# tzt101/MichiGAN

Hardware: AMD Instinct MI355X
Metric: training images/sec at 512x512 (G+D step) (higher is better)
Workload: dtype bf16; 1 GPU; SPADEB G + multiscale PatchGAN D + VGG19 + Gabor orientation losses, full G step + D step (Adam), bs=8/GPU, 512x512, BASELINE.json configs[2]; global_batch=8, batch_per_gpu=8, resolution=512, parallelism=dp1, init=reference default (xavier, 0.02), random VGG weights

## Files before the change

### michigan_amd/csrc/mg_wgrad3x3.hip

```cpp
#include "mg_conv_common.h"
#include "mg_wgrad_common.h"


namespace {

typedef __attribute__((ext_vector_type(4))) short s16x4_t;
typedef __attribute__((ext_vector_type(8))) short s16x8_t;
typedef __attribute__((address_space(3))) s16x4_t* lds_s16x4_p;

__device__ unsigned long long* g_mg_wg3_probe_out = nullptr;
__device__ __forceinline__ unsigned long long wg3_stamp()
{
    unsigned long long v;
    asm volatile("s_memrealtime %0\n\ts_waitcnt lgkmcnt(0)" : "=s"(v) :: "memory");
    return v;
}

template <int MT, int NT, bool W16, bool PROBE = false>
__global__ __launch_bounds__(256, 2) void wgrad3x3_kernel(const Wg3K d)
{
    constexpr int TM = 64 * MT, TN = 64 * NT;
    constexpr int RBA = TM * 2, RBB = TN * 2;
    constexpr int PPA = RBA / 16, PPB = RBB / 16;
    constexpr int A_ROWS = 32, B_ROWS = (NT == 2) ? 36 : 40;
    constexpr int A_BYTES = A_ROWS * RBA, B_BYTES = B_ROWS * RBB;
    constexpr int A_IPS = A_BYTES / 4096;
    constexpr int B_IPS = (B_BYTES + 4095) / 4096;
    constexpr int IPS = A_IPS + B_IPS;
    constexpr int STAGE = A_BYTES + B_BYTES;
    constexpr int NS = 4;
    static_assert(A_BYTES % 4096 == 0 && B_BYTES % 1024 == 0, "stage must be whole wave blocks");

    extern __shared__ __attribute__((aligned(16))) unsigned char smem[];

    const int tid = threadIdx.x, lane = tid & 63;
    const int wave = __builtin_amdgcn_readfirstlane(tid >> 6);
    const int wm = wave >> 1, wn = wave & 1;
    const int l31 = lane & 31, hi = lane >> 5;

    int tile;
    {
        const int nblk = gridDim.x, b = blockIdx.x;
        const int q8 = nblk >> 3, r8 = nblk & 7, xcd = b & 7, idx = b >> 3;
        tile = (xcd < r8 ? xcd * (q8 + 1) : r8 * (q8 + 1) + (xcd - r8) * q8) + idx;
    }
    const int tm = tile % d.tiles_m;  tile /= d.tiles_m;
    const int tn = tile % d.tiles_n;  tile /= d.tiles_n;
    const int ky = tile % 3;
    const int split = tile / 3;
    const int m0 = tm * TM, n0 = tn * TN;
    const int sbeg = split * d.sps;
    const int send = min(d.nstg, sbeg + d.sps);
    const int nk = send - sbeg;
    if (nk <= 0) return;

    const int H = d.H, W = d.W;
    constexpr int SEG = W16 ? 16 : 32, SEGP = SEG + 2;
    constexpr int PR = (32 / SEG) * SEGP;
    const unsigned lds0 = (unsigned)(size_t)(__attribute__((address_space(3))) unsigned char*)smem;
    const unsigned dump = lds0 + NS * STAGE + wave * 1024;
    const unsigned char* zsrc = g_mg_zeros + (lane & 3) * 16;

    auto swz_a = [](int row) { return RBA == 256 ? (row & 3) : ((row >> 1) & 1); };
    auto swz_b = [](int row) { return RBB == 256 ? (row & 3) : ((row >> 1) & 1); };

    int aoff[A_IPS];
#pragma unroll
    for (int j = 0; j < A_IPS; ++j) {
        const int g = j * 256 + tid, row = g / PPA, slot = g % PPA;
        int ch = m0 + ((slot ^ (swz_a(row) << 2)) << 3);
        if (ch >= d.Cg) ch = m0;
        aoff[j] = (row * d.Cg + ch) * 2;
    }
    int boff[B_IPS], brc[B_IPS];
#pragma unroll
    for (int j = 0; j < B_IPS; ++j) {
        const int g = j * 256 + tid, row = g / PPB, slot = g % PPB;
        int ch = n0 + ((slot ^ (swz_b(row) << 2)) << 3);
        if (ch >= d.Cin) ch = n0;
        const int r = (W16 && row >= SEGP) ? 1 : 0, c = row - r * SEGP - 1;
        boff[j] = (((r + ky - 1) * W + c) * d.Cin + ch) * 2;
        brc[j] = row < PR ? (r | (c + 1) << 4) : -1;
    }
    const unsigned char* const dy0 = reinterpret_cast<const unsigned char*>(d.dy);
    const unsigned char* const x0p = reinterpret_cast<const unsigned char*>(d.x);
    const unsigned char* abase; const unsigned char* xbase;
    int sy, sx, sg_next = sbeg;
    int simg = 0, sstripe = 0;
    const int SWp = W16 ? W : d.stripe_w, nsegs = SWp / 32, nstripes = W / SWp;
    if (W16) {
        abase = dy0 + (size_t)sbeg * 32 * d.Cg * 2;
        xbase = x0p + (size_t)sbeg * 32 * d.Cin * 2;
        const int rem = (sbeg * 32) % (H * W); sy = rem / W; sx = rem - sy * W;
    } else {
        const int spi = H * (W / 32);
        simg = sbeg / spi;
        int r = sbeg - simg * spi;
        sstripe = r / (H * nsegs);  r -= sstripe * (H * nsegs);
        sy = r / nsegs;
        sx = sstripe * SWp + (r - sy * nsegs) * 32;
        const size_t p = ((size_t)simg * H + sy) * W + sx;
        abase = dy0 + p * d.Cg * 2;
        xbase = x0p + p * d.Cin * 2;
    }
    sy = __builtin_amdgcn_readfirstlane(sy); sx = __builtin_amdgcn_readfirstlane(sx);
    simg = __builtin_amdgcn_readfirstlane(simg); sstripe = __builtin_amdgcn_readfirstlane(sstripe);
    const int a_step = 32 * d.Cg * 2, x_step = 32 * d.Cin * 2;

    unsigned long long m_live[B_IPS], m_left[B_IPS], m_right[B_IPS], m_r1[B_IPS];
#pragma unroll
    for (int j = 0; j < B_IPS; ++j) {
        const bool lv = brc[j] >= 0;
        const int c = (brc[j] >> 4) - 1, r = brc[j] & 15;
        m_live[j]  = __builtin_amdgcn_ballot_w64(lv);
        m_left[j]  = __builtin_amdgcn_ballot_w64(lv && c == -1);
        m_right[j] = __builtin_amdgcn_ballot_w64(lv && c == SEG);
        m_r1[j]    = __builtin_amdgcn_ballot_w64(lv && r == 1);
    }
    const unsigned long long zaddr = (unsigned long long)(size_t)zsrc;
    const unsigned zlo = (unsigned)zaddr, zhi = (unsigned)(zaddr >> 32);

    auto issue = [&](int stage) {
        const bool real = sg_next < send;
        const unsigned sbase = lds0 + stage * STAGE;
        if (real) {
#pragma unroll
            for (int j = 0; j < A_IPS; ++j)
                glds16_s(abase, (unsigned)aoff[j], __builtin_amdgcn_readfirstlane(sbase + j * 4096 + wave * 1024));
        } else {
#pragma unroll
            for (int j = 0; j < A_IPS; ++j)
                glds16(zsrc, __builtin_amdgcn_readfirstlane(sbase + j * 4096 + wave * 1024));
        }
        const int sxs = __builtin_amdgcn_readfirstlane(sx), sys = __builtin_amdgcn_readfirstlane(sy), kys = __builtin_amdgcn_readfirstlane(ky);
        const bool lok = sxs > 0, rok = sxs + SEG < W;
        const bool y0 = (unsigned)(sys + kys - 1) < (unsigned)H, y1 = (unsigned)(sys + kys) < (unsigned)H;
#pragma unroll
        for (int j = 0; j < B_IPS; ++j) {
            unsigned long long v = real ? m_live[j] : 0ull;
            if (!lok) v &= ~m_left[j];
            if (!rok) v &= ~m_right[j];
            if (W16) { if (!y0) v &= m_r1[j]; if (!y1) v &= ~m_r1[j]; }
            else if (!y0) v = 0ull;
            v = ((unsigned long long)(unsigned)__builtin_amdgcn_readfirstlane((int)(v >> 32)) << 32) | (unsigned)__builtin_amdgcn_readfirstlane((int)v);
            asm("" : "+s"(v));
            const unsigned long long pa = (unsigned long long)(size_t)(xbase + boff[j]);
            unsigned plo, phi;
            asm("v_cndmask_b32_e64 %0, %1, %2, %3" : "=v"(plo) : "v"(zlo), "v"((unsigned)pa), "s"(v));
            asm("v_cndmask_b32_e64 %0, %1, %2, %3" : "=v"(phi) : "v"(zhi), "v"((unsigned)(pa >> 32)), "s"(v));
            const bool live = (j * 4096 + wave * 1024) < B_BYTES;
            glds16(reinterpret_cast<const void*>((size_t)(((unsigned long long)phi << 32) | plo)),
                   __builtin_amdgcn_readfirstlane(live ? sbase + A_BYTES + j * 4096 + wave * 1024 : dump));
        }
        ++sg_next;
        if (W16) {
            abase += a_step; xbase += x_step;
            sy += 2; if (sy >= H) sy = 0;
        } else {
            sx += 32;
            if (sx < (sstripe + 1) * SWp) { abase += a_step; xbase += x_step; }
            else {
                sx = sstripe * SWp; ++sy;
                if (sy >= H) { sy = 0; ++sstripe; if (sstripe >= nstripes) { sstripe = 0; ++simg; } sx = sstripe * SWp; }
                const size_t p = ((size_t)simg * H + sy) * W + sx;
                abase = dy0 + p * d.Cg * 2;
                xbase = x0p + p * d.Cin * 2;
            }
        }
    };

    f32x16_t acc[3][MT][NT];
#pragma unroll
    for (int kx = 0; kx < 3; ++kx)
#pragma unroll
        for (int mt = 0; mt < MT; ++mt)
#pragma unroll
            for (int nt = 0; nt < NT; ++nt)
#pragma unroll
                for (int r = 0; r < 16; ++r) acc[kx][mt][nt][r] = 0.f;

    const bool do_bias = d.dbias != nullptr && ky == 1 && tn == 0 && wn == 0;
    float bsum[MT];
#pragma unroll
    for (int mt = 0; mt < MT; ++mt) bsum[mt] = 0.f;

    const int i16 = lane & 15, g2 = lane >> 4;
    const int rsub = (g2 >> 1) * 8 + (i16 >> 2);
    const int csub = ((g2 & 1) * 16 + (i16 & 3) * 4) * 2;
    constexpr int ksb = W16 ? SEGP : 16;

    auto compute = [&](int slot) {
        const unsigned char* As = smem + slot * STAGE;
        const unsigned char* Bs = As + A_BYTES;
#pragma unroll
        for (int ks = 0; ks < 2; ++ks) {
            bf16x8_t a[MT];
            const int ra = ks * 16 + rsub;
#pragma unroll
            for (int mt = 0; mt < MT; ++mt) {
                const int col = ((wm * MT + mt) * 64 + csub) ^ (swz_a(ra) << 6);
                const unsigned char* p = As + ra * RBA + col;
                s16x4_t v0 = __builtin_amdgcn_ds_read_tr16_b64_v4i16((lds_s16x4_p)(p));
                s16x4_t v1 = __builtin_amdgcn_ds_read_tr16_b64_v4i16((lds_s16x4_p)(p + 4 * RBA));
                a[mt] = __builtin_bit_cast(bf16x8_t, __builtin_shufflevector(v0, v1, 0, 1, 2, 3, 4, 5, 6, 7));
                if (do_bias) {
                    typedef __attribute__((ext_vector_type(4))) unsigned u32x4_t;
                    const u32x4_t w = __builtin_bit_cast(u32x4_t, a[mt]);
#pragma unroll
                    for (int j = 0; j < 4; ++j) bsum[mt] += __uint_as_float(w[j] << 16) + __uint_as_float(w[j] & 0xffff0000u);
                }
            }
            static_for<0, 3>([&](auto kx_) {
                constexpr int kx = decltype(kx_)::value;
                bf16x8_t b[NT];
                const int rb = ks * ksb + kx + rsub;
#pragma unroll
                for (int nt = 0; nt < NT; ++nt) {
                    const int col = ((wn * NT + nt) * 64 + csub) ^ (swz_b(rb) << 6);
                    const unsigned char* p = Bs + rb * RBB + col;
                    s16x4_t v0 = __builtin_amdgcn_ds_read_tr16_b64_v4i16((lds_s16x4_p)(p));
                    s16x4_t v1 = __builtin_amdgcn_ds_read_tr16_b64_v4i16((lds_s16x4_p)(p + 4 * RBB));
                    b[nt] = __builtin_bit_cast(bf16x8_t, __builtin_shufflevector(v0, v1, 0, 1, 2, 3, 4, 5, 6, 7));
                }
#pragma unroll
                for (int mt = 0; mt < MT; ++mt)
#pragma unroll
                    for (int nt = 0; nt < NT; ++nt)
                        acc[kx][mt][nt] = __builtin_amdgcn_mfma_f32_32x32x16_bf16(a[mt], b[nt], acc[kx][mt][nt], 0, 0, 0);
            });
        }
    };

#pragma unroll
    for (int s = 0; s < NS - 1; ++s) issue(s);
    int slot = 0, islot = NS - 1;
    unsigned long long t_wait = 0, t_bar = 0, t_issue = 0, t_mfma = 0, t_begin = 0;
    if constexpr (PROBE) t_begin = wg3_stamp();
    for (int it = 0; it < nk; ++it) {
        unsigned long long s0 = 0, s1 = 0, s2 = 0, s3 = 0;
        if constexpr (PROBE) s0 = wg3_stamp();
        wait_vmcnt<(NS - 2) * IPS>();
        if constexpr (PROBE) s1 = wg3_stamp();
        __builtin_amdgcn_s_barrier();
        if constexpr (PROBE) s2 = wg3_stamp();
        issue(islot);
        if constexpr (PROBE) s3 = wg3_stamp();
        compute(slot);
        if constexpr (PROBE) { const unsigned long long s4 = wg3_stamp(); t_wait += s1 - s0; t_bar += s2 - s1; t_issue += s3 - s2; t_mfma += s4 - s3; }
        slot = (slot == NS - 1) ? 0 : slot + 1;
        islot = (islot == NS - 1) ? 0 : islot + 1;
    }
    wait_vmcnt<0>();
    unsigned long long t_loop_end = 0;
    if constexpr (PROBE) t_loop_end = wg3_stamp();

    if (do_bias) {
#pragma unroll
        for (int mt = 0; mt < MT; ++mt) {
            const float t = bsum[mt] + __shfl_xor(bsum[mt], 32);
            const int co = m0 + (wm * MT + mt) * 32 + l31;
            if (hi == 0 && co < d.Cg) wg_accum(d.dbias, d.det_stride, split, (size_t)co, t);
        }
    }

    static_for<0, 3 * MT * NT>([&](auto i_) {
        constexpr int kx = decltype(i_)::value / (MT * NT), mt = (decltype(i_)::value / NT) % MT, nt = decltype(i_)::value % NT;
        const int ci = n0 + (wn * NT + nt) * 32 + l31;
        if (ci >= d.Cin) return;
        const int tap = ky * 3 + kx;
#pragma unroll
        for (int r = 0; r < 16; ++r) {
            const int co = m0 + (wm * MT + mt) * 32 + (r & 3) + 8 * (r >> 2) + 4 * hi;
            if (co < d.Cg)
                wg_accum(d.dw, d.det_stride, split, (size_t)(tap * d.Cg + co) * d.Cin + ci, acc[kx][mt][nt][r]);
        }
    });
    if constexpr (PROBE) {
        const unsigned long long t_end = wg3_stamp();
        if (lane == 0 && g_mg_wg3_probe_out) {
            unsigned long long* o = g_mg_wg3_probe_out + ((size_t)blockIdx.x * 4 + wave) * 8;
            o[0] = t_wait; o[1] = t_bar; o[2] = t_issue; o[3] = t_mfma; o[4] = t_loop_end - t_begin; o[5] = t_end - t_loop_end; o[6] = (unsigned long long)nk; o[7] = t_begin;
        }
    }
}


template <int MT, int NT, bool W16>
int launch3(Wg3K& k, hipStream_t st, int* nsplit, bool dry)
{
    constexpr int TM = 64 * MT, TN = 64 * NT;
    constexpr int STAGE = 32 * TM * 2 + ((NT == 2) ? 36 : 40) * TN * 2;
    constexpr size_t LDS = 4 * (size_t)STAGE + 4096;
    k.tiles_m = (k.Cg + TM - 1) / TM;
    k.tiles_n = (k.Cin + TN - 1) / TN;
    const int stripe = mg_opt(MG_OPT_WGRAD3X3_STRIPE);
    k.stripe_w = (!W16 && stripe >= 32 && (stripe % 32) == 0 && k.W > stripe && (k.W % stripe) == 0) ? stripe : k.W;
    const long base = 3L * k.tiles_m * k.tiles_n;
    int S = k.splitk;
    if (S <= 0) {
        const int lo = (int)((384 + base - 1) / base), hi = (int)((1536 + base - 1) / base);
        S = k.nstg / 192 < hi ? k.nstg / 192 : hi;
        if (S < lo) S = lo;
        if (S > k.nstg / 16) S = k.nstg / 16;
        if (S < 1) S = 1;
    }
    if (S > k.nstg) S = k.nstg;
    k.sps = (k.nstg + S - 1) / S;
    S = (k.nstg + k.sps - 1) / k.sps;
    const long nblk = base * S;
    if (nsplit) *nsplit = S;
    if (dry) return MG_OK;
    if (nblk <= 0 || nblk > 0x7fffffffL) return mg_fail(MG_ERR_ARG, "mg_conv_wgrad: bad grid %ld", nblk);
    auto kern = wgrad3x3_kernel<MT, NT, W16>;
    constexpr size_t LDS_HALF_CU = LDS > 84 * 1024 ? LDS : 84 * 1024;
    const size_t lds_req = k.half_cu ? LDS_HALF_CU : LDS;
    mg_raise_lds_cap(reinterpret_cast<const void*>(kern), (int)LDS_HALF_CU);
#if MG_PROBES
    if constexpr (MT == 2 && NT == 2 && !W16) {
        if (mg_opt(MG_OPT_PROBE_WGRAD3X3)) {
            auto pk = wgrad3x3_kernel<MT, NT, W16, true>;
            mg_raise_lds_cap(reinterpret_cast<const void*>(pk), (int)LDS);
            hipLaunchKernelGGL(pk, dim3((unsigned)nblk), dim3(256), LDS, st, k);
            MG_CHECK_LAUNCH("mg_conv_wgrad(3x3 probe)");
            return MG_OK;
        }
    }
#endif
    hipLaunchKernelGGL(kern, dim3((unsigned)nblk), dim3(256), lds_req, st, k);
    MG_CHECK_LAUNCH("mg_conv_wgrad(3x3)");
    return MG_OK;
}

}

int wgrad3x3_set_probe(unsigned long long addr)
{
    unsigned long long* p = reinterpret_cast<unsigned long long*>(addr);
    return hipMemcpyToSymbol(HIP_SYMBOL(g_mg_wg3_probe_out), &p, sizeof(p)) == hipSuccess ? MG_OK : MG_ERR_ARG;
}

int launch_wgrad3x3(Wg3K& k, hipStream_t st, int* nsplit, bool dry)
{
    const bool m2 = k.Cg > 64, n2 = k.Cin > 64;
    if (k.W == 16) {
        if (m2 && n2) return launch3<2, 2, true>(k, st, nsplit, dry);
        if (m2)       return launch3<2, 1, true>(k, st, nsplit, dry);
        if (n2)       return launch3<1, 2, true>(k, st, nsplit, dry);
        return launch3<1, 1, true>(k, st, nsplit, dry);
    }
    if (m2 && n2) return launch3<2, 2, false>(k, st, nsplit, dry);
    if (m2)       return launch3<2, 1, false>(k, st, nsplit, dry);
    if (n2)       return launch3<1, 2, false>(k, st, nsplit, dry);
    return launch3<1, 1, false>(k, st, nsplit, dry);
}
```

Before: 131.8 images/s.

## Add nine-tap 3x3 weight-gradient kernel reusing input rows across ky taps

For W != 16, 3x3 weight-gradient convolutions now go to a new kernel. Each block computes all nine taps for a 64x64 tile. Input rows stream through a ring of LDS stages, so the three ky taps reuse the previous, current and next rows already in LDS, and the kx shift is formed in registers with alignbit instead of separate loads. This removes the separate grid dimension over ky and the threefold reloading of x and dy. The cost is nine accumulator tiles per wave (high register pressure), a fixed 64x64 tile, and a different split-K heuristic.

```diff
diff --git a/michigan_amd/csrc/mg_wgrad3x3.hip b/michigan_amd/csrc/mg_wgrad3x3.hip
--- a/michigan_amd/csrc/mg_wgrad3x3.hip
+++ b/michigan_amd/csrc/mg_wgrad3x3.hip
@@ -7,6 +7,7 @@
 typedef __attribute__((ext_vector_type(4))) short s16x4_t;
 typedef __attribute__((ext_vector_type(8))) short s16x8_t;
 typedef __attribute__((address_space(3))) s16x4_t* lds_s16x4_p;
+typedef __attribute__((ext_vector_type(4))) unsigned u32x4_t;
 
 __device__ unsigned long long* g_mg_wg3_probe_out = nullptr;
 __device__ __forceinline__ unsigned long long wg3_stamp()
@@ -16,7 +17,258 @@
     return v;
 }
 
-template <int MT, int NT, bool W16, bool PROBE = false>
+template <int RB>
+__device__ __forceinline__ bf16x8_t wg3_frag(const unsigned char* p)
+{
+    s16x4_t v0 = __builtin_amdgcn_ds_read_tr16_b64_v4i16((lds_s16x4_p)(p));
+    s16x4_t v1 = __builtin_amdgcn_ds_read_tr16_b64_v4i16((lds_s16x4_p)(p + 4 * RB));
+    return __builtin_bit_cast(bf16x8_t, __builtin_shufflevector(v0, v1, 0, 1, 2, 3, 4, 5, 6, 7));
+}
+
+__device__ __forceinline__ float wg3_sum8(bf16x8_t a)
+{
+    const u32x4_t w = __builtin_bit_cast(u32x4_t, a);
+    float s = 0.f;
+#pragma unroll
+    for (int j = 0; j < 4; ++j) s += __uint_as_float(w[j] << 16) + __uint_as_float(w[j] & 0xffff0000u);
+    return s;
+}
+
+__device__ __forceinline__ int wg3_tile()
+{
+    const int nblk = gridDim.x, b = blockIdx.x;
+    const int q8 = nblk >> 3, r8 = nblk & 7, xcd = b & 7, idx = b >> 3;
+    return (xcd < r8 ? xcd * (q8 + 1) : r8 * (q8 + 1) + (xcd - r8) * q8) + idx;
+}
+
+struct Wg9 {
+    static constexpr int RB = 128;
+    static constexpr int A_BYTES = 32 * RB;
+    static constexpr int B_BYTES = 40 * RB;
+    static constexpr int STAGE = A_BYTES + B_BYTES;
+    static constexpr int IPS = 3;
+    static constexpr int PF = 3;
+    static constexpr int NS = PF + 3;
+    static constexpr int DUMP = NS * STAGE, ZERO = DUMP + 4096;
+    static constexpr int LDS = ZERO + B_BYTES;
+};
+
+template <bool PROBE>
+__global__ __launch_bounds__(256, 2) void wgrad3x3_ninetap_kernel(const Wg3K d)
+{
+    constexpr int RB = Wg9::RB, A_BYTES = Wg9::A_BYTES, B_BYTES = Wg9::B_BYTES, STAGE = Wg9::STAGE, NS = Wg9::NS, PF = Wg9::PF;
+    constexpr int LIVE = 34;
+
+    extern __shared__ __attribute__((aligned(16))) unsigned char smem[];
+
+    const int tid = threadIdx.x, lane = tid & 63;
+    const int wave = __builtin_amdgcn_readfirstlane(tid >> 6);
+    const int wm = wave >> 1, wn = wave & 1;
+    const int l31 = lane & 31, hi = lane >> 5;
+
+    int tile = wg3_tile();
+    const int tm = tile % d.tiles_m;  tile /= d.tiles_m;
+    const int tn = tile % d.tiles_n;
+    const int split = tile / d.tiles_n;
+    const int m0 = tm * 64, n0 = tn * 64;
+    const int sbeg = split * d.sps;
+    const int send = min(d.nstg, sbeg + d.sps);
+    const int nk = send - sbeg;
+    if (nk <= 0) return;
+
+    const int H = d.H, W = d.W, nstripes = W / 32;
+    const unsigned lds0 = (unsigned)(size_t)(__attribute__((address_space(3))) unsigned char*)smem;
+    const unsigned dump = lds0 + Wg9::DUMP + wave * 1024;
+    const unsigned char* zsrc = g_mg_zeros + (lane & 3) * 16;
+
+    auto swz = [](int row) { return (row >> 1) & 1; };
+
+    int aoff, boff[2];
+    bool blive[2];
+    {
+        const int row = tid >> 3, slot = tid & 7;
+        int ch = m0 + ((slot ^ (swz(row) << 2)) << 3);
+        if (ch >= d.Cg) ch = m0;
+        aoff = (row * d.Cg + ch) * 2;
+    }
+#pragma unroll
+    for (int j = 0; j < 2; ++j) {
+        const int g = j * 256 + tid, row = g >> 3, slot = g & 7;
+        int ch = n0 + ((slot ^ (swz(row) << 2)) << 3);
+        if (ch >= d.Cin) ch = n0;
+        boff[j] = ((row - 1) * d.Cin + ch) * 2;
+        blive[j] = row < LIVE;
+    }
+    unsigned long long m_live[2], m_left[2], m_right[2];
+#pragma unroll
+    for (int j = 0; j < 2; ++j) {
+        const int row = (j * 256 + tid) >> 3;
+        m_live[j]  = __builtin_amdgcn_ballot_w64(blive[j]);
+        m_left[j]  = __builtin_amdgcn_ballot_w64(blive[j] && row == 0);
+        m_right[j] = __builtin_amdgcn_ballot_w64(blive[j] && row == LIVE - 1);
+    }
+    const unsigned long long zaddr = (unsigned long long)(size_t)zsrc;
+    const unsigned zlo = (unsigned)zaddr, zhi = (unsigned)(zaddr >> 32);
+
+    const unsigned char* const dy0 = reinterpret_cast<const unsigned char*>(d.dy);
+    const unsigned char* const x0p = reinterpret_cast<const unsigned char*>(d.x);
+    const int a_row = W * d.Cg * 2, x_row = W * d.Cin * 2;
+    int an = sbeg, ay, astripe, aimg;
+    int xs = sbeg - 1, xy, xstripe, ximg;
+    const int xlast = min(send, d.nstg - 1);
+    {
+        int is = sbeg / H;
+        ay = sbeg - is * H; aimg = is / nstripes; astripe = is - aimg * nstripes;
+        const int x1 = max(xs, 0);
+        is = x1 / H;
+        xy = x1 - is * H; ximg = is / nstripes; xstripe = is - ximg * nstripes;
+    }
+    ay = __builtin_amdgcn_readfirstlane(ay); astripe = __builtin_amdgcn_readfirstlane(astripe); aimg = __builtin_amdgcn_readfirstlane(aimg);
+    xy = __builtin_amdgcn_readfirstlane(xy); xstripe = __builtin_amdgcn_readfirstlane(xstripe); ximg = __builtin_amdgcn_readfirstlane(ximg);
+    const unsigned char* abase = dy0 + (((size_t)aimg * H + ay) * W + astripe * 32) * d.Cg * 2;
+    const unsigned char* xbase = x0p + (((size_t)ximg * H + xy) * W + xstripe * 32) * d.Cin * 2;
+
+    auto issue_a = [&](unsigned sbase) {
+        const unsigned dst = __builtin_amdgcn_readfirstlane(sbase + wave * 1024);
+        if (an < send) glds16_s(abase, (unsigned)aoff, dst);
+        else glds16(zsrc, dst);
+        ++an; ++ay;
+        if (ay < H) abase += a_row;
+        else {
+            ay = 0; ++astripe;
+            if (astripe >= nstripes) { astripe = 0; ++aimg; }
+            abase = dy0 + ((size_t)aimg * H * W + astripe * 32) * d.Cg * 2;
+        }
+    };
+    auto issue_b = [&](unsigned bbase) {
+        const bool real = xs >= 0 && xs <= xlast;
+        const int sxs = __builtin_amdgcn_readfirstlane(xstripe) * 32;
+        const bool lok = sxs > 0, rok = sxs + 32 < W;
+#pragma unroll
+        for (int j = 0; j < 2; ++j) {
+            unsigned long long v = real ? m_live[j] : 0ull;
+            if (!lok) v &= ~m_left[j];
+            if (!rok) v &= ~m_right[j];
+            v = ((unsigned long long)(unsigned)__builtin_amdgcn_readfirstlane((int)(v >> 32)) << 32) | (unsigned)__builtin_amdgcn_readfirstlane((int)v);
+            asm("" : "+s"(v));
+            const unsigned long long pa = (unsigned long long)(size_t)(xbase + boff[j]);
+            unsigned plo, phi;
+            asm("v_cndmask_b32_e64 %0, %1, %2, %3" : "=v"(plo) : "v"(zlo), "v"((unsigned)pa), "s"(v));
+            asm("v_cndmask_b32_e64 %0, %1, %2, %3" : "=v"(phi) : "v"(zhi), "v"((unsigned)(pa >> 32)), "s"(v));
+            const bool inside = (j * 4096 + wave * 1024) < B_BYTES;
+            glds16(reinterpret_cast<const void*>((size_t)(((unsigned long long)phi << 32) | plo)),
+                   __builtin_amdgcn_readfirstlane(inside ? bbase + j * 4096 + wave * 1024 : dump));
+        }
+        if (real) {
+            ++xy;
+            if (xy < H) xbase += x_row;
+            else {
+                xy = 0; ++xstripe;
+                if (xstripe >= nstripes) { xstripe = 0; ++ximg; }
+                xbase = x0p + ((size_t)ximg * H * W + xstripe * 32) * d.Cin * 2;
+            }
+        }
+        ++xs;
+    };
+
+    f32x16_t acc[9];
+#pragma unroll
+    for (int t = 0; t < 9; ++t)
+#pragma unroll
+        for (int r = 0; r < 16; ++r) acc[t][r] = 0.f;
+
+    const bool do_bias = d.dbias != nullptr && tn == 0 && wn == 0;
+    float bsum = 0.f;
+
+    const int i16 = lane & 15, g2 = lane >> 4;
+    const int rsub = (g2 >> 1) * 8 + (i16 >> 2);
+    const int csub = ((g2 & 1) * 16 + (i16 & 3) * 4) * 2;
+
+    auto compute = [&](const unsigned char* As, const unsigned char* B0, const unsigned char* B1, const unsigned char* B2) {
+#pragma unroll
+        for (int ks = 0; ks < 2; ++ks) {
+            const int ra = ks * 16 + rsub;
+            const bf16x8_t a = wg3_frag<RB>(As + ra * RB + ((wm * 64 + csub) ^ (swz(ra) << 6)));
+            if (do_bias) bsum += wg3_sum8(a);
+            static_for<0, 3>([&](auto ky_) {
+                constexpr int ky = decltype(ky_)::value;
+                const unsigned char* Bs = ky == 0 ? B0 : ky == 1 ? B1 : B2;
+                const int r0 = ks * 16 + rsub, r2 = r0 + 2;
+                const bf16x8_t b0 = wg3_frag<RB>(Bs + r0 * RB + ((wn * 64 + csub) ^ (swz(r0) << 6)));
+                const bf16x8_t b2 = wg3_frag<RB>(Bs + r2 * RB + ((wn * 64 + csub) ^ (swz(r2) << 6)));
+                const u32x4_t u0 = __builtin_bit_cast(u32x4_t, b0), u2 = __builtin_bit_cast(u32x4_t, b2);
+                u32x4_t u1;
+#pragma unroll
+                for (int i = 0; i < 4; ++i) u1[i] = __builtin_amdgcn_alignbit(i < 3 ? u0[(i + 1) & 3] : u2[3], u0[i], 16);
+                acc[ky * 3 + 0] = __builtin_amdgcn_mfma_f32_32x32x16_bf16(a, b0, acc[ky * 3 + 0], 0, 0, 0);
+                acc[ky * 3 + 1] = __builtin_amdgcn_mfma_f32_32x32x16_bf16(a, __builtin_bit_cast(bf16x8_t, u1), acc[ky * 3 + 1], 0, 0, 0);
+                acc[ky * 3 + 2] = __builtin_amdgcn_mfma_f32_32x32x16_bf16(a, b2, acc[ky * 3 + 2], 0, 0, 0);
+            });
+        }
+    };
+
+    glds16(zsrc, __builtin_amdgcn_readfirstlane(lds0 + Wg9::ZERO + wave * 1024));
+    glds16(zsrc, __builtin_amdgcn_readfirstlane(wave == 0 ? lds0 + Wg9::ZERO + 4096 : dump));
+    issue_b(lds0 + 0 * STAGE + A_BYTES);
+    issue_b(lds0 + 1 * STAGE + A_BYTES);
+#pragma unroll
+    for (int s = 2; s < PF + 2; ++s) { issue_a(lds0 + s * STAGE); issue_b(lds0 + s * STAGE + A_BYTES); }
+    int s0 = 0, s1 = 1, s2 = 2, islot = NS - 1;
+    int cy = __builtin_amdgcn_readfirstlane(sbeg % H);
+    unsigned long long t_wait = 0, t_bar = 0, t_issue = 0, t_mfma = 0, t_begin = 0;
+    if constexpr (PROBE) t_begin = wg3_stamp();
+    for (int it = 0; it < nk; ++it) {
+        unsigned long long p0 = 0, p1 = 0, p2 = 0, p3 = 0;
+        if constexpr (PROBE) p0 = wg3_stamp();
+        wait_vmcnt<(PF - 1) * Wg9::IPS>();
+        if constexpr (PROBE) p1 = wg3_stamp();
+        __builtin_amdgcn_s_barrier();
+        if constexpr (PROBE) p2 = wg3_stamp();
+        issue_a(lds0 + islot * STAGE); issue_b(lds0 + islot * STAGE + A_BYTES);
+        if constexpr (PROBE) p3 = wg3_stamp();
+        const unsigned char* const zs = smem + Wg9::ZERO;
+        compute(smem + s2 * STAGE,
+                cy == 0 ? zs : smem + s0 * STAGE + A_BYTES,
+                smem + s1 * STAGE + A_BYTES,
+                cy == H - 1 ? zs : smem + s2 * STAGE + A_BYTES);
+        if constexpr (PROBE) { const unsigned long long p4 = wg3_stamp(); t_wait += p1 - p0; t_bar += p2 - p1; t_issue += p3 - p2; t_mfma += p4 - p3; }
+        s0 = s1; s1 = s2;
+        s2 = (s2 == NS - 1) ? 0 : s2 + 1;
+        islot = (islot == NS - 1) ? 0 : islot + 1;
+        cy = (cy == H - 1) ? 0 : cy + 1;
+    }
+    wait_vmcnt<0>();
+    unsigned long long t_loop_end = 0;
+    if constexpr (PROBE) t_loop_end = wg3_stamp();
+
+    if (do_bias) {
+        const float t = bsum + __shfl_xor(bsum, 32);
+        const int co = m0 + wm * 32 + l31;
+        if (hi == 0 && co < d.Cg) wg_accum(d.dbias, d.det_stride, split, (size_t)co, t);
+    }
+
+    const int ci = n0 + wn * 32 + l31;
+    if (ci < d.Cin) {
+        static_for<0, 9>([&](auto t_) {
+            constexpr int tap = decltype(t_)::value;
+#pragma unroll
+            for (int r = 0; r < 16; ++r) {
+                const int co = m0 + wm * 32 + (r & 3) + 8 * (r >> 2) + 4 * hi;
+                if (co < d.Cg)
+                    wg_accum(d.dw, d.det_stride, split, (size_t)(tap * d.Cg + co) * d.Cin + ci, acc[tap][r]);
+            }
+        });
+    }
+    if constexpr (PROBE) {
+        const unsigned long long t_end = wg3_stamp();
+        if (lane == 0 && g_mg_wg3_probe_out) {
+            unsigned long long* o = g_mg_wg3_probe_out + ((size_t)blockIdx.x * 4 + wave) * 8;
+            o[0] = t_wait; o[1] = t_bar; o[2] = t_issue; o[3] = t_mfma; o[4] = t_loop_end - t_begin; o[5] = t_end - t_loop_end; o[6] = (unsigned long long)nk; o[7] = t_begin;
+        }
+    }
+}
+
+template <int MT, int NT>
 __global__ __launch_bounds__(256, 2) void wgrad3x3_kernel(const Wg3K d)
 {
     constexpr int TM = 64 * MT, TN = 64 * NT;
@@ -38,12 +290,7 @@
     const int wm = wave >> 1, wn = wave & 1;
     const int l31 = lane & 31, hi = lane >> 5;
 
-    int tile;
-    {
-        const int nblk = gridDim.x, b = blockIdx.x;
-        const int q8 = nblk >> 3, r8 = nblk & 7, xcd = b & 7, idx = b >> 3;
-        tile = (xcd < r8 ? xcd * (q8 + 1) : r8 * (q8 + 1) + (xcd - r8) * q8) + idx;
-    }
+    int tile = wg3_tile();
     const int tm = tile % d.tiles_m;  tile /= d.tiles_m;
     const int tn = tile % d.tiles_n;  tile /= d.tiles_n;
     const int ky = tile % 3;
@@ -55,8 +302,8 @@
     if (nk <= 0) return;
 
     const int H = d.H, W = d.W;
-    constexpr int SEG = W16 ? 16 : 32, SEGP = SEG + 2;
-    constexpr int PR = (32 / SEG) * SEGP;
+    constexpr int SEG = 16, SEGP = SEG + 2;
+    constexpr int PR = 2 * SEGP;
     const unsigned lds0 = (unsigned)(size_t)(__attribute__((address_space(3))) unsigned char*)smem;
     const unsigned dump = lds0 + NS * STAGE + wave * 1024;
     const unsigned char* zsrc = g_mg_zeros + (lane & 3) * 16;
@@ -78,44 +325,23 @@
         const int g = j * 256 + tid, row = g / PPB, slot = g % PPB;
         int ch = n0 + ((slot ^ (swz_b(row) << 2)) << 3);
         if (ch >= d.Cin) ch = n0;
-        const int r = (W16 && row >= SEGP) ? 1 : 0, c = row - r * SEGP - 1;
+        const int r = row >= SEGP ? 1 : 0, c = row - r * SEGP - 1;
         boff[j] = (((r + ky - 1) * W + c) * d.Cin + ch) * 2;
         brc[j] = row < PR ? (r | (c + 1) << 4) : -1;
     }
-    const unsigned char* const dy0 = reinterpret_cast<const unsigned char*>(d.dy);
-    const unsigned char* const x0p = reinterpret_cast<const unsigned char*>(d.x);
-    const unsigned char* abase; const unsigned char* xbase;
-    int sy, sx, sg_next = sbeg;
-    int simg = 0, sstripe = 0;
-    const int SWp = W16 ? W : d.stripe_w, nsegs = SWp / 32, nstripes = W / SWp;
-    if (W16) {
-        abase = dy0 + (size_t)sbeg * 32 * d.Cg * 2;
-        xbase = x0p + (size_t)sbeg * 32 * d.Cin * 2;
-        const int rem = (sbeg * 32) % (H * W); sy = rem / W; sx = rem - sy * W;
-    } else {
-        const int spi = H * (W / 32);
-        simg = sbeg / spi;
-        int r = sbeg - simg * spi;
-        sstripe = r / (H * nsegs);  r -= sstripe * (H * nsegs);
-        sy = r / nsegs;
-        sx = sstripe * SWp + (r - sy * nsegs) * 32;
-        const size_t p = ((size_t)simg * H + sy) * W + sx;
-        abase = dy0 + p * d.Cg * 2;
-        xbase = x0p + p * d.Cin * 2;
-    }
-    sy = __builtin_amdgcn_readfirstlane(sy); sx = __builtin_amdgcn_readfirstlane(sx);
-    simg = __builtin_amdgcn_readfirstlane(simg); sstripe = __builtin_amdgcn_readfirstlane(sstripe);
+    const unsigned char* abase = reinterpret_cast<const unsigned char*>(d.dy) + (size_t)sbeg * 32 * d.Cg * 2;
+    const unsigned char* xbase = reinterpret_cast<const unsigned char*>(d.x) + (size_t)sbeg * 32 * d.Cin * 2;
+    int sy = ((sbeg * 32) % (H * W)) / W, sg_next = sbeg;
+    sy = __builtin_amdgcn_readfirstlane(sy);
     const int a_step = 32 * d.Cg * 2, x_step = 32 * d.Cin * 2;
 
-    unsigned long long m_live[B_IPS], m_left[B_IPS], m_right[B_IPS], m_r1[B_IPS];
+    unsigned long long m_live[B_IPS], m_r1[B_IPS];
 #pragma unroll
     for (int j = 0; j < B_IPS; ++j) {
-        const bool lv = brc[j] >= 0;
         const int c = (brc[j] >> 4) - 1, r = brc[j] & 15;
-        m_live[j]  = __builtin_amdgcn_ballot_w64(lv);
-        m_left[j]  = __builtin_amdgcn_ballot_w64(lv && c == -1);
-        m_right[j] = __builtin_amdgcn_ballot_w64(lv && c == SEG);
-        m_r1[j]    = __builtin_amdgcn_ballot_w64(lv && r == 1);
+        const bool lv = brc[j] >= 0 && c != -1 && c != SEG;
+        m_live[j] = __builtin_amdgcn_ballot_w64(lv);
+        m_r1[j]   = __builtin_amdgcn_ballot_w64(lv && r == 1);
     }
     const unsigned long long zaddr = (unsigned long long)(size_t)zsrc;
     const unsigned zlo = (unsigned)zaddr, zhi = (unsigned)(zaddr >> 32);
@@ -132,16 +358,13 @@
             for (int j = 0; j < A_IPS; ++j)
                 glds16(zsrc, __builtin_amdgcn_readfirstlane(sbase + j * 4096 + wave * 1024));
         }
-        const int sxs = __builtin_amdgcn_readfirstlane(sx), sys = __builtin_amdgcn_readfirstlane(sy), kys = __builtin_amdgcn_readfirstlane(ky);
-        const bool lok = sxs > 0, rok = sxs + SEG < W;
+        const int sys = __builtin_amdgcn_readfirstlane(sy), kys = __builtin_amdgcn_readfirstlane(ky);
         const bool y0 = (unsigned)(sys + kys - 1) < (unsigned)H, y1 = (unsigned)(sys + kys) < (unsigned)H;
 #pragma unroll
         for (int j = 0; j < B_IPS; ++j) {
             unsigned long long v = real ? m_live[j] : 0ull;
-            if (!lok) v &= ~m_left[j];
-            if (!rok) v &= ~m_right[j];
-            if (W16) { if (!y0) v &= m_r1[j]; if (!y1) v &= ~m_r1[j]; }
-            else if (!y0) v = 0ull;
+            if (!y0) v &= m_r1[j];
+            if (!y1) v &= ~m_r1[j];
             v = ((unsigned long long)(unsigned)__builtin_amdgcn_readfirstlane((int)(v >> 32)) << 32) | (unsigned)__builtin_amdgcn_readfirstlane((int)v);
             asm("" : "+s"(v));
             const unsigned long long pa = (unsigned long long)(size_t)(xbase + boff[j]);
@@ -153,20 +376,8 @@
                    __builtin_amdgcn_readfirstlane(live ? sbase + A_BYTES + j * 4096 + wave * 1024 : dump));
         }
         ++sg_next;
-        if (W16) {
-            abase += a_step; xbase += x_step;
-            sy += 2; if (sy >= H) sy = 0;
-        } else {
-            sx += 32;
-            if (sx < (sstripe + 1) * SWp) { abase += a_step; xbase += x_step; }
-            else {
-                sx = sstripe * SWp; ++sy;
-                if (sy >= H) { sy = 0; ++sstripe; if (sstripe >= nstripes) { sstripe = 0; ++simg; } sx = sstripe * SWp; }
-                const size_t p = ((size_t)simg * H + sy) * W + sx;
-                abase = dy0 + p * d.Cg * 2;
-                xbase = x0p + p * d.Cin * 2;
-            }
-        }
+        abase += a_step; xbase += x_step;
+        sy += 2; if (sy >= H) sy = 0;
     };
 
     f32x16_t acc[3][MT][NT];
@@ -187,7 +398,7 @@
     const int i16 = lane & 15, g2 = lane >> 4;
     const int rsub = (g2 >> 1) * 8 + (i16 >> 2);
     const int csub = ((g2 & 1) * 16 + (i16 & 3) * 4) * 2;
-    constexpr int ksb = W16 ? SEGP : 16;
+    constexpr int ksb = SEGP;
 
     auto compute = [&](int slot) {
         const unsigned char* As = smem + slot * STAGE;
@@ -198,30 +409,16 @@
             const int ra = ks * 16 + rsub;
 #pragma unroll
             for (int mt = 0; mt < MT; ++mt) {
-                const int col = ((wm * MT + mt) * 64 + csub) ^ (swz_a(ra) << 6);
-                const unsigned char* p = As + ra * RBA + col;
-                s16x4_t v0 = __builtin_amdgcn_ds_read_tr16_b64_v4i16((lds_s16x4_p)(p));
-                s16x4_t v1 = __builtin_amdgcn_ds_read_tr16_b64_v4i16((lds_s16x4_p)(p + 4 * RBA));
-                a[mt] = __builtin_bit_cast(bf16x8_t, __builtin_shufflevector(v0, v1, 0, 1, 2, 3, 4, 5, 6, 7));
-                if (do_bias) {
-                    typedef __attribute__((ext_vector_type(4))) unsigned u32x4_t;
-                    const u32x4_t w = __builtin_bit_cast(u32x4_t, a[mt]);
-#pragma unroll
-                    for (int j = 0; j < 4; ++j) bsum[mt] += __uint_as_float(w[j] << 16) + __uint_as_float(w[j] & 0xffff0000u);
-                }
+                a[mt] = wg3_frag<RBA>(As + ra * RBA + (((wm * MT + mt) * 64 + csub) ^ (swz_a(ra) << 6)));
+                if (do_bias) bsum[mt] += wg3_sum8(a[mt]);
             }
             static_for<0, 3>([&](auto kx_) {
                 constexpr int kx = decltype(kx_)::value;
                 bf16x8_t b[NT];
                 const int rb = ks * ksb + kx + rsub;
 #pragma unroll
-                for (int nt = 0; nt < NT; ++nt) {
-                    const int col = ((wn * NT + nt) * 64 + csub) ^ (swz_b(rb) << 6);
-                    const unsigned char* p = Bs + rb * RBB + col;
-                    s16x4_t v0 = __builtin_amdgcn_ds_read_tr16_b64_v4i16((lds_s16x4_p)(p));
-                    s16x4_t v1 = __builtin_amdgcn_ds_read_tr16_b64_v4i16((lds_s16x4_p)(p + 4 * RBB));
-                    b[nt] = __builtin_bit_cast(bf16x8_t, __builtin_shufflevector(v0, v1, 0, 1, 2, 3, 4, 5, 6, 7));
-                }
+                for (int nt = 0; nt < NT; ++nt)
+                    b[nt] = wg3_frag<RBB>(Bs + rb * RBB + (((wn * NT + nt) * 64 + csub) ^ (swz_b(rb) << 6)));
 #pragma unroll
                 for (int mt = 0; mt < MT; ++mt)
 #pragma unroll
@@ -234,25 +431,15 @@
 #pragma unroll
     for (int s = 0; s < NS - 1; ++s) issue(s);
     int slot = 0, islot = NS - 1;
-    unsigned long long t_wait = 0, t_bar = 0, t_issue = 0, t_mfma = 0, t_begin = 0;
-    if constexpr (PROBE) t_begin = wg3_stamp();
     for (int it = 0; it < nk; ++it) {
-        unsigned long long s0 = 0, s1 = 0, s2 = 0, s3 = 0;
-        if constexpr (PROBE) s0 = wg3_stamp();
         wait_vmcnt<(NS - 2) * IPS>();
-        if constexpr (PROBE) s1 = wg3_stamp();
         __builtin_amdgcn_s_barrier();
-        if constexpr (PROBE) s2 = wg3_stamp();
         issue(islot);
-        if constexpr (PROBE) s3 = wg3_stamp();
         compute(slot);
-        if constexpr (PROBE) { const unsigned long long s4 = wg3_stamp(); t_wait += s1 - s0; t_bar += s2 - s1; t_issue += s3 - s2; t_mfma += s4 - s3; }
         slot = (slot == NS - 1) ? 0 : slot + 1;
         islot = (islot == NS - 1) ? 0 : islot + 1;
     }
     wait_vmcnt<0>();
-    unsigned long long t_loop_end = 0;
-    if constexpr (PROBE) t_loop_end = wg3_stamp();
 
     if (do_bias) {
 #pragma unroll
@@ -275,17 +462,56 @@
                 wg_accum(d.dw, d.det_stride, split, (size_t)(tap * d.Cg + co) * d.Cin + ci, acc[kx][mt][nt][r]);
         }
     });
-    if constexpr (PROBE) {
-        const unsigned long long t_end = wg3_stamp();
-        if (lane == 0 && g_mg_wg3_probe_out) {
-            unsigned long long* o = g_mg_wg3_probe_out + ((size_t)blockIdx.x * 4 + wave) * 8;
-            o[0] = t_wait; o[1] = t_bar; o[2] = t_issue; o[3] = t_mfma; o[4] = t_loop_end - t_begin; o[5] = t_end - t_loop_end; o[6] = (unsigned long long)nk; o[7] = t_begin;
-        }
-    }
-}
-
-
-template <int MT, int NT, bool W16>
+}
+
+
+int wg3_splits(Wg3K& k, long base, int slots_lo, int slots_hi, int long_split)
+{
+    int S = k.splitk;
+    if (S <= 0) {
+        const int lo = (int)((slots_lo + base - 1) / base), hi = (int)((slots_hi + base - 1) / base);
+        S = k.nstg / long_split < hi ? k.nstg / long_split : hi;
+        if (S < lo) S = lo;
+        if (S > k.nstg / 16) S = k.nstg / 16;
+        if (S < 1) S = 1;
+    }
+    if (S > k.nstg) S = k.nstg;
+    k.sps = (k.nstg + S - 1) / S;
+    return (k.nstg + k.sps - 1) / k.sps;
+}
+
+constexpr size_t wg3_half_cu_lds(size_t lds) { return lds > 84 * 1024 ? lds : 84 * 1024; }
+
+int launch9(Wg3K& k, hipStream_t st, int* nsplit, bool dry)
+{
+    k.tiles_m = (k.Cg + 63) / 64;
+    k.tiles_n = (k.Cin + 63) / 64;
+    k.stripe_w = 32;
+    const long base = (long)k.tiles_m * k.tiles_n;
+    const int S = wg3_splits(k, base, 512, 512, 256);
+    const long nblk = base * S;
+    if (nsplit) *nsplit = S;
+    if (dry) return MG_OK;
+    if (nblk <= 0 || nblk > 0x7fffffffL) return mg_fail(MG_ERR_ARG, "mg_conv_wgrad: bad grid %ld", nblk);
+    constexpr size_t LDS = Wg9::LDS, LDS_HALF_CU = wg3_half_cu_lds(LDS);
+    const size_t lds_req = k.half_cu ? LDS_HALF_CU : LDS;
+    auto kern = wgrad3x3_ninetap_kernel<false>;
+    mg_raise_lds_cap(reinterpret_cast<const void*>(kern), (int)LDS_HALF_CU);
+#if MG_PROBES
+    if (mg_opt(MG_OPT_PROBE_WGRAD3X3)) {
+        auto pk = wgrad3x3_ninetap_kernel<true>;
+        mg_raise_lds_cap(reinterpret_cast<const void*>(pk), (int)LDS);
+        hipLaunchKernelGGL(pk, dim3((unsigned)nblk), dim3(256), LDS, st, k);
+        MG_CHECK_LAUNCH("mg_conv_wgrad(3x3 probe)");
+        return MG_OK;
+    }
+#endif
+    hipLaunchKernelGGL(kern, dim3((unsigned)nblk), dim3(256), lds_req, st, k);
+    MG_CHECK_LAUNCH("mg_conv_wgrad(3x3 nine-tap)");
+    return MG_OK;
+}
+
+template <int MT, int NT>
 int launch3(Wg3K& k, hipStream_t st, int* nsplit, bool dry)
 {
     constexpr int TM = 64 * MT, TN = 64 * NT;
@@ -293,39 +519,17 @@
     constexpr size_t LDS = 4 * (size_t)STAGE + 4096;
     k.tiles_m = (k.Cg + TM - 1) / TM;
     k.tiles_n = (k.Cin + TN - 1) / TN;
-    const int stripe = mg_opt(MG_OPT_WGRAD3X3_STRIPE);
-    k.stripe_w = (!W16 && stripe >= 32 && (stripe % 32) == 0 && k.W > stripe && (k.W % stripe) == 0) ? stripe : k.W;
+    k.stripe_w = k.W;
     const long base = 3L * k.tiles_m * k.tiles_n;
-    int S = k.splitk;
-    if (S <= 0) {
-        const int lo = (int)((384 + base - 1) / base), hi = (int)((1536 + base - 1) / base);
-        S = k.nstg / 192 < hi ? k.nstg / 192 : hi;
-        if (S < lo) S = lo;
-        if (S > k.nstg / 16) S = k.nstg / 16;
-        if (S < 1) S = 1;
-    }
-    if (S > k.nstg) S = k.nstg;
-    k.sps = (k.nstg + S - 1) / S;
-    S = (k.nstg + k.sps - 1) / k.sps;
+    const int S = wg3_splits(k, base, 384, 1536, 192);
     const long nblk = base * S;
     if (nsplit) *nsplit = S;
     if (dry) return MG_OK;
     if (nblk <= 0 || nblk > 0x7fffffffL) return mg_fail(MG_ERR_ARG, "mg_conv_wgrad: bad grid %ld", nblk);
-    auto kern = wgrad3x3_kernel<MT, NT, W16>;
-    constexpr size_t LDS_HALF_CU = LDS > 84 * 1024 ? LDS : 84 * 1024;
+    auto kern = wgrad3x3_kernel<MT, NT>;
+    constexpr size_t LDS_HALF_CU = wg3_half_cu_lds(LDS);
     const size_t lds_req = k.half_cu ? LDS_HALF_CU : LDS;
     mg_raise_lds_cap(reinterpret_cast<const void*>(kern), (int)LDS_HALF_CU);
-#if MG_PROBES
-    if constexpr (MT == 2 && NT == 2 && !W16) {
-        if (mg_opt(MG_OPT_PROBE_WGRAD3X3)) {
-            auto pk = wgrad3x3_kernel<MT, NT, W16, true>;
-            mg_raise_lds_cap(reinterpret_cast<const void*>(pk), (int)LDS);
-            hipLaunchKernelGGL(pk, dim3((unsigned)nblk), dim3(256), LDS, st, k);
-            MG_CHECK_LAUNCH("mg_conv_wgrad(3x3 probe)");
-            return MG_OK;
-        }
-    }
-#endif
     hipLaunchKernelGGL(kern, dim3((unsigned)nblk), dim3(256), lds_req, st, k);
     MG_CHECK_LAUNCH("mg_conv_wgrad(3x3)");
     return MG_OK;
@@ -341,15 +545,10 @@
 
 int launch_wgrad3x3(Wg3K& k, hipStream_t st, int* nsplit, bool dry)
 {
+    if (k.W != 16) return launch9(k, st, nsplit, dry);
     const bool m2 = k.Cg > 64, n2 = k.Cin > 64;
-    if (k.W == 16) {
-        if (m2 && n2) return launch3<2, 2, true>(k, st, nsplit, dry);
-        if (m2)       return launch3<2, 1, true>(k, st, nsplit, dry);
-        if (n2)       return launch3<1, 2, true>(k, st, nsplit, dry);
-        return launch3<1, 1, true>(k, st, nsplit, dry);
-    }
-    if (m2 && n2) return launch3<2, 2, false>(k, st, nsplit, dry);
-    if (m2)       return launch3<2, 1, false>(k, st, nsplit, dry);
-    if (n2)       return launch3<1, 2, false>(k, st, nsplit, dry);
-    return launch3<1, 1, false>(k, st, nsplit, dry);
-}
+    if (m2 && n2) return launch3<2, 2>(k, st, nsplit, dry);
+    if (m2)       return launch3<2, 1>(k, st, nsplit, dry);
+    if (n2)       return launch3<1, 2>(k, st, nsplit, dry);
+    return launch3<1, 1>(k, st, nsplit, dry);
+}
```

New measurement: 132.6 images/s, median of 6. No clear change (+0.6%).
